# bobu36000/gym-chess

Hardware: NVIDIA B200
Metric: env_steps_per_sec (higher is better)
Workload: dtype u64

## Files before the change

__graft_entry__.py:

```python
import os
import subprocess
import sys

ROOT = os.path.dirname(os.path.abspath(__file__))
if ROOT not in sys.path:
    sys.path.insert(0, ROOT)


def build():
    from gym_chess_b200 import _lib

    _lib.build_all(force=True)
    subprocess.check_call(["make", "-C", os.path.join(ROOT, "oracle"), "-s", "-B"])
    from tests.host_emul import emul

    emul.build(force=True)
    from tests.host_emul import clone_emul

    clone_emul.build(force=True)
    import gym_chess_b200

    L = _lib.lib()
    assert L.gcb_version() >= 100


def smoke():
    import numpy as np

    from gym_chess_b200 import BatchedChessEngine, BatchedChessEnv
    from oracle import oracle as orc

    N, T, seed = 64, 40, 7
    env = BatchedChessEnv(N, opponent="none", seed=seed, device=0)
    O = [orc.OracleEnv(seed=seed, env_id=i) for i in range(N)]

    def oracle_step(i, o):
        v = o.view()
        rr, dd, _ = o.step(o.pick(orc.draw_u32(seed, i, v["episode"], v["step_in_episode"], 0)))
        if dd or o.view()["n_legal"] == 0:
            o.reset(v["episode"] + 1)
        return rr, dd

# ... 29 lines not shown
```

gym_chess_b200/csrc/chess_core.cuh:

```cuda
#pragma once
#include <stdint.h>

typedef unsigned long long u64;
typedef unsigned int u32;

#ifndef GCB_ROLL_NTH
#define GCB_ROLL_NTH 1
#endif

#if defined(__CUDACC__)
#define GCB_HD __host__ __device__ __forceinline__
#else
#define GCB_HD inline
#endif

GCB_HD u64 gcb_brev64(u64 x) {
#if defined(__CUDA_ARCH__)
    return __brevll(x);
#else
    x = ((x >> 1) & 0x5555555555555555ULL) | ((x & 0x5555555555555555ULL) << 1);
    x = ((x >> 2) & 0x3333333333333333ULL) | ((x & 0x3333333333333333ULL) << 2);
    x = ((x >> 4) & 0x0F0F0F0F0F0F0F0FULL) | ((x & 0x0F0F0F0F0F0F0F0FULL) << 4);
    return __builtin_bswap64(x);
#endif
// ... 369 lines not shown
    const u64 cand = (eRQ & (geo.line(ksq, 0) | geo.line(ksq, 1))) | (eBQ & (geo.line(ksq, 2) | geo.line(ksq, 3)));
    for (u64 p = cand; p;) {
        const int psq = gcb_take(p);
        const u64 btw = GCB_GEOM(between[ksq][psq]), blockers = btw & occ;
        if (!blockers) chk |= 1ULL << psq;
        else if (!(blockers & (blockers - 1)) && (blockers & g.own)) g.pinned |= blockers, g.pinrays |= btw | (1ULL << psq);
    }
    g.in_check = chk != 0;
    if (chk) {
        if (chk & (chk - 1)) g.cm = 0;
        else g.cm = chk | GCB_GEOM(between[ksq][gcb_lsb(chk)]);
    }
    (void)kbit;
}

GCB_HD void gen_prepare(const Board& b, int white_to_move, GenCtx& g) { gen_prepare(b, white_to_move, g, GeomGlobal()); }

GCB_HD u64 pin_mask(const GenCtx& g, int sq) {
    const u64 kbit = 1ULL << g.ksq;
    const u64 side = sq > g.ksq ? ~(kbit | (kbit - 1)) : (kbit - 1);
    return g.pinrays & line_through(g.ksq, sq) & side;
}

template <class Sink, class G>
GCB_HD void gen_targets(const Board& b, GenCtx& g, u64 subset, Sink& sink, const G& geo) {
    const u64 occ = g.occ, own = g.own, notown = ~g.own;
    const u64 mine = own & subset;
#define GCB_PUT(sq_, below_, T_)                                       \
    do {                                                               \
        const u64 t__ = (T_);                                          \
        sink.put(gcb_popc(mine & (below_)), t__);                      \
    } while (0)
    for (u64 s = bb_rooks(b) & mine; s;) {
        u64 below;
        const int sq = gcb_take(s, below);
        const u64 a = rook_att(geo, sq, occ);
        g.satt |= a;
        GCB_PUT(sq, below, a & notown & g.cm);
    }
    for (u64 s = bb_bishops(b) & mine; s;) {
        u64 below;
        const int sq = gcb_take(s, below);
        const u64 a = bishop_att(geo, sq, occ);
        g.satt |= a;
        GCB_PUT(sq, below, a & notown & g.cm);
    }
    for (u64 s = bb_queens(b) & mine; s;) {
        u64 below;
        const int sq = gcb_take(s, below);
        const u64 a = rook_att(geo, sq, occ) | bishop_att(geo, sq, occ);
        g.satt |= a;
        GCB_PUT(sq, below, a & notown & g.cm);
    }
    for (u64 s = bb_knights(b) & mine; s;) {
        u64 below;
        const int sq = gcb_take(s, below);
        const u64 a = geo.knight(sq);
        g.satt |= a;
        GCB_PUT(sq, below, a & notown & g.cm);
    }
    for (u64 s = bb_kings(b) & mine; s;) {
        u64 below;
        const int sq = gcb_take(s, below);
        const u64 a = geo.king(sq);
        g.satt |= a;
        GCB_PUT(sq, below, a & notown & ~g.eatt);
    }
    {
        const u64 pw = bb_pawns(b) & mine, allp = bb_pawns(b) & own;
        g.satt |= pawn_set_att(pw, g.white) & ~(bb_kings(b) & own);
        (void)allp;
        const u64 free_cm = ~occ & g.cm, enemy_cm = g.enemy & g.cm;
        for (u64 s = pw; s;) {
            u64 below;
            const int sq = gcb_take(s, below);
            const u64 push = geo.pawn(!g.white, sq, 0), cap = geo.pawn(!g.white, sq, 1);
            GCB_PUT(sq, below, (push & free_cm) | (cap & enemy_cm));
        }
    }
#undef GCB_PUT
    for (u64 p = g.pinned & mine & ~bb_kings(b); p;) {
        u64 below;
        const int sq = gcb_take(p, below), r = gcb_popc(mine & below);
        const u64 t = sink.get(r), t2 = t & pin_mask(g, sq);
        sink.replace(r, t, t2);
    }
}

template <class Sink>
GCB_HD void gen_targets(const Board& b, GenCtx& g, u64 subset, Sink& sink) {
    gen_targets(b, g, subset, sink, GeomGlobal());
}

GCB_HD u32 gen_castles(const Board& b, const GenCtx& g, u32 rights) {
    if (!g.has_king) return 0;
    const u64 wR = bb_rooks(b) & b.w, wK = bb_kings(b) & b.w, occ = g.occ, eatt = g.eatt;
    u32 c = 0;
    if (g.white) {
        if (!(rights & (RT_WK | RT_WQ))) return 0;
        const u64 e1 = 1ULL << 60;
        if ((wR >> 56 & 1) && !(occ & (7ULL << 57)) && (wK & e1) && !(eatt & (7ULL << 58))) c |= 1u;
        if ((wR >> 63 & 1) && !(occ & (3ULL << 61)) && (wK & e1) && !(eatt & (7ULL << 60))) c |= 2u;
    } else {
        if (!(rights & (RT_BK | RT_BQ))) return 0;
        const u64 e8 = 1ULL << 4;
        if ((wR & 1) && !(occ & (7ULL << 1)) && (wK & e8) && !(eatt & (7ULL << 2))) c |= 1u;
        if ((wR >> 7 & 1) && !(occ & (3ULL << 5)) && (wK & e8) && !(eatt & (7ULL << 4))) c |= 2u;
    }
    return c;
}
GCB_HD int castle_action(int white, int king_side) {
    return white ? (king_side ? ACT_CASTLE_KS_WHITE : ACT_CASTLE_QS_WHITE) : (king_side ? ACT_CASTLE_KS_BLACK : ACT_CASTLE_QS_BLACK);
}

// ... 426 lines not shown
```

gym_chess_b200/csrc/env_core.cuh:

```cuda
#pragma once
#include "chess_core.cuh"

#if !defined(__CUDACC__)
struct ulonglong2 {
    u64 x, y;
};
static inline ulonglong2 make_ulonglong2(u64 x, u64 y) {
    ulonglong2 r = {x, y};
    return r;
}
#endif

#if defined(__CUDACC__)
__device__ unsigned long long g_violations = 0ULL;
#endif
#if defined(GCB_CHECKED) && defined(__CUDA_ARCH__)
#define GCB_CHK(cond, code)                                                   \
    do {                                                                      \
        if (!(cond)) atomicOr(&g_violations, 1ULL << (code));                 \
    } while (0)
#else
#define GCB_CHK(cond, code) \
    do {                    \
    } while (0)
// ... 41 lines not shown
#define M_MOVECOUNT_SHIFT 22
#define M_STEP_SHIFT 38
#define M_HIST_SHIFT 54

enum { ST_STEPS = 0, ST_PLIES, ST_EPISODES, ST_MATES, ST_REPS, ST_CAPS, ST_WEDGED, ST_INVALID, ST_REWARD, ST_LEGAL,
       ST_INCHECK, ST_HISTOVF, ST_SLOTOVF, ST_HISTSCAN, ST_WINDOW, ST_USED, ST_COUNT = 16 };

struct EnvView {
    ulonglong2* bb01;
    ulonglong2* bb23;
    u64* meta;
    u64* zkey;
    u32* gen;
    ulonglong2* rep;
    u32* episode;
    ulonglong2* cnt;
    u64* tgt;
    const ulonglong2* t_bb01;
    const ulonglong2* t_bb23;
    const u64* t_meta;
    const u64* t_zkey;
    const u64* t_tgt;
    const ulonglong2* t_cnt;
    const u64* zob;
    u64* stats;
    u64* stat_rows;
    u64 seed;
    int N, slots, hist_mask, n_templates, stat_nrows;
    u32 env_offset;
    int moves_max, opponent, agent_black, auto_reset, pps;
};

struct EnvRegs {
    Board b;
    u64 zk, cnt_lo, cnt_hi;
    u32 rights, chk, castle;
    int stm_black, done, n_legal, move_count, step, hist_len, pending;
    u32 gen;
};

GCB_HD void unpack_meta(u64 m, EnvRegs& s) {
    s.stm_black = (int)(m & 1);
    s.rights = (u32)(m >> M_RIGHTS_SHIFT) & 15u;
    s.chk = (u32)(m >> 5) & 3u;
    s.done = (int)(m >> 7) & 1;
    s.castle = (u32)(m >> M_CASTLE_SHIFT) & 3u;
// ... 74 lines not shown
    }
};

struct TgtSinkFast {
    u64* base;
    unsigned N;
    int dropped;
    uint8_t* cb;
    GCB_HD TgtSinkFast(const SlotRef& sr, CountBytes* scratch) : base(sr.base), N(sr.stride), dropped(0), cb(scratch->c) {
        u64* z = reinterpret_cast<u64*>(scratch);
        z[0] = 0, z[1] = 0;
    }
    GCB_HD void put(int r, u64 t) {
        GCB_CHK((unsigned)r < 16u, CHK_SLOT_INDEX);
        base[(unsigned)r * N] = t;
        cb[r] = (uint8_t)gcb_popc(t);
    }
    GCB_HD u64 get(int r) const { return base[(unsigned)r * N]; }
    GCB_HD void replace(int r, u64, u64 tnew) {
        GCB_CHK((unsigned)r < 16u, CHK_SLOT_INDEX);
        base[(unsigned)r * N] = tnew;
        cb[r] = (uint8_t)gcb_popc(tnew);
    }
    GCB_HD u64 count_lo() const { return reinterpret_cast<const u64*>(cb)[0]; }
    GCB_HD u64 count_hi() const { return reinterpret_cast<const u64*>(cb)[1]; }
    GCB_HD int total() const {
        u64 a = count_lo(), b = count_hi();
        a = (a & 0x00FF00FF00FF00FFULL) + ((a >> 8) & 0x00FF00FF00FF00FFULL);
        b = (b & 0x00FF00FF00FF00FFULL) + ((b >> 8) & 0x00FF00FF00FF00FFULL);
        a += b;
        a += a >> 32;
        a += a >> 16;
        return (int)(a & 0xFFFF);
    }
};

struct StepStats {
    u32 f;
    int reward, legal, scan, window;
    bool wrote_slots;
    GCB_HD void clear() { f = 0, reward = 0, legal = 0, scan = 0, window = 0, wrote_slots = false; }
    GCB_HD int get(int k) const {
        switch (k) {
        case ST_STEPS: return (int)(f & 127u);
        case ST_PLIES: return (int)((f >> 7) & 255u);
        case ST_EPISODES: return (int)((f >> 22) & 1u);
        case ST_MATES: return (int)((f >> 23) & 1u);
        case ST_REPS: return (int)((f >> 24) & 1u);
        case ST_CAPS: return (int)((f >> 25) & 1u);
        case ST_WEDGED: return (int)((f >> 26) & 1u);
        case ST_INVALID: return (int)((f >> 27) & 1u);
        case ST_REWARD: return reward;
        case ST_LEGAL: return legal;
        case ST_INCHECK: return (int)((f >> 15) & 127u);
        case ST_HISTOVF: return (int)((f >> 28) & 3u);
        case ST_SLOTOVF: return (int)((f >> 30) & 3u);
        case ST_HISTSCAN: return scan;
        default: return window;
// ... 52 lines not shown
            const u64 c = (en.y & 3ULL) < 3ULL ? (en.y & 3ULL) + 1ULL : 3ULL;
            if (insert) GCB_STS(p, make_ulonglong2(key, live_tag | c));
            return (int)c;
        }
        st.scan++;
    }
    st.f += SF_HISTOVF;
    if (insert) GCB_STS(&tab[home], make_ulonglong2(key, live_tag | 1ULL));
    return 1;
}

#ifndef GCB_ONE_PICK_SITE
#define GCB_ONE_PICK_SITE 1
#endif
#ifndef GCB_SWAR_PICK
#define GCB_SWAR_PICK 1
#endif
GCB_HD u64 swar_le_u8(u64 x, u64 y) {
    const u64 H = 0x8080808080808080ULL;
    const u64 t = (y | H) - (x & ~H);
    return ((~x & y) | (~(x ^ y) & t)) & H;
}

template <bool ROLLED = true>
GCB_HD int action_at(const SlotRef& sr, const EnvRegs& s, int idx) {
    int acc = 0, hit_r = -1, hit_idx = 0;
#if GCB_SWAR_PICK
    if (s.n_legal <= 255) {
        const u64 K = 0x0101010101010101ULL;
        const u64 p_lo = s.cnt_lo * K, p_hi = (s.cnt_hi + (p_lo >> 56)) * K;
        const u64 I = (u64)(u32)idx * K;
        const int r = gcb_popc(swar_le_u8(p_lo, I)) + gcb_popc(swar_le_u8(p_hi, I));
        acc = (int)(p_hi >> 56);
        if (r < 16) {
            const u64 q = r < 8 ? (p_lo << 8) : ((p_hi << 8) | (p_lo >> 56));
            hit_r = r, hit_idx = idx - (int)((q >> (8 * (r & 7))) & 0xFF);
        }
    } else
#endif
    {
#if defined(__CUDA_ARCH__)
#pragma unroll 1
#endif
        for (int r = 0; r < 16; r++) {
            const int c = (int)(((r < 8 ? s.cnt_lo : s.cnt_hi) >> (8 * (r & 7))) & 0xFF);
            if (hit_r < 0 && idx - acc < c) hit_r = r, hit_idx = idx - acc;
            acc += c;
        }
    }
    TgtSink slots(sr, nullptr);
    u64 own = stm_pieces(s);
    if (sr.slots > 16 && hit_r < 0) {
        const int np = gcb_popc(own);
        for (int r = 16; r < np && hit_r < 0; r++) {
            const int c = gcb_popc(slots.get(r));
            if (idx - acc < c) hit_r = r, hit_idx = idx - acc;
            else acc += c;
        }
    }
    if (hit_r >= 0) {
        const u64 T = slots.get(hit_r);
        const int sq = gcb_select64(own, hit_r);
        return sq * 64 + nth_target<ROLLED>(piece_code(s.b, sq), !s.stm_black, sq, T, hit_idx);
    }
    const int king_side = (s.castle & 1u) ? (idx - acc != 0) : 1;
    return castle_action(!s.stm_black, king_side);
}

GCB_HD bool action_is_legal(const SlotRef& sr, const EnvRegs& s, int action) {
    if (action < 0) return false;
    if (action < 4096) {
        const int from = action >> 6, to = action & 63;
        const u64 own = stm_pieces(s), fbit = 1ULL << from;
        if (!(own & fbit)) return false;
        TgtSink slots(sr, nullptr);
        return (slots.get(gcb_popc(own & (fbit - 1))) >> to) & 1ULL;
    }
    if (action == castle_action(!s.stm_black, 0)) return s.castle & 1u;
    if (action == castle_action(!s.stm_black, 1)) return (s.castle >> 1) & 1u;
    return false;
}



template <bool FAST> struct SinkOf { typedef TgtSink type; };
template <> struct SinkOf<true> { typedef TgtSinkFast type; };

template <bool FAST = false, class G>
GCB_HD int ply_and_movegen(const EnvView& v, int e, EnvRegs& s, int action, bool apply, bool* rep,
                           StepStats& st, CountBytes* scratch, const SlotRef& sr, const G& geo) {
    int r = 0;
    *rep = false;
    if (apply) {
        const u64 key = hist_key(s.zk);
        u32 rights = mask_rights(s.b, s.rights);
        int status;
        bool irr;
        r = apply_action(s.b, rights, !s.stm_black, action, &status, &irr, &s.zk, v.zob);
        s.rights = rights;
        st.window += s.hist_len;
        *rep = rep_lookup_insert(v, e, s, key, !irr, st) >= 3;
        if (irr) {
            s.hist_len = 0, s.gen++;
        } else {
            if (s.hist_len < 0x1FF) s.hist_len++;
        }
    }
    s.stm_black ^= 1;
    GenCtx g;
    gen_prepare(s.b, !s.stm_black, g, geo);
    typename SinkOf<FAST>::type sink(sr, scratch);
    gen_targets(s.b, g, g.own, sink, geo);
    st.wrote_slots = true;
    const int n = sink.total();
    if (sink.dropped) st.f += SF_SLOTOVF;
    s.cnt_lo = sink.count_lo(), s.cnt_hi = sink.count_hi();
    s.castle = gen_castles(s.b, g, mask_rights(s.b, s.rights));
    s.n_legal = n + (int)(s.castle & 1u) + (int)(s.castle >> 1);
    u32 chk = g.in_check ? (1u << s.stm_black) : 0u;
    const u64 mk = bb_kings(s.b) & g.enemy;
    if (mk && ((g.satt >> ref_king_square(mk)) & 1ULL)) chk |= 1u << (s.stm_black ^ 1);
    s.chk = chk;
    return r;
}

enum { MODE_ACTION = 0, MODE_INDEX = 1, MODE_SAMPLED = 2, MODE_RESET = 3, MODE_BOTPLY = 4 };
enum { PH_AGENT = 0, PH_BOT = 1, PH_FINAL = 2, PH_RESETBOT = 3, PH_END = 4 };

struct StepIO {
    const void* in;
    int32_t* reward;
    uint8_t* done;
    uint8_t* flags;
    int32_t* act_out;
    int32_t* bot_out;
// ... 19 lines not shown

GCB_HD void env_load(const EnvView& v, int e, EnvRegs& s, u32& ep) {
    GCB_CHK((unsigned)e < (unsigned)v.N, CHK_ENV_INDEX);
    ulonglong2 a = GCB_LDS(&v.bb01[e]), c = GCB_LDS(&v.bb23[e]);
    s.b.t0 = a.x, s.b.t1 = a.y, s.b.t2 = c.x, s.b.w = c.y;
    ulonglong2 ct = GCB_LDS(&v.cnt[e]);
    s.cnt_lo = ct.x, s.cnt_hi = ct.y;
    unpack_meta(GCB_LDS(&v.meta[e]), s);
    s.zk = GCB_LDS(&v.zkey[e]);
    ep = GCB_LDS(&v.episode[e]);
    s.gen = GCB_LDS(&v.gen[e]);
}
GCB_HD void env_store(const EnvView& v, int e, const EnvRegs& s, u32 ep) {
    GCB_CHK((unsigned)e < (unsigned)v.N, CHK_ENV_INDEX);
    GCB_STS(&v.bb01[e], make_ulonglong2(s.b.t0, s.b.t1));
    GCB_STS(&v.bb23[e], make_ulonglong2(s.b.t2, s.b.w));
    GCB_STS(&v.cnt[e], make_ulonglong2(s.cnt_lo, s.cnt_hi));
    GCB_STS(&v.meta[e], pack_meta(s));
    GCB_STS(&v.zkey[e], s.zk);
    GCB_STS(&v.episode[e], ep);
    GCB_STS(&v.gen[e], s.gen);
}

template <int MODE, bool SELFPLAY = false, bool FAST = false, bool MULTI = false, class G>
GCB_HD void env_step_regs(const EnvView& v, const StepIO& io, int e, EnvRegs& s, u32& ep, StepStats& st, CountBytes* scratch,
                          const SlotRef& sr, const SlotRef& pick_sr, const G& geo, const u32 input) {
    const bool v_bot = SELFPLAY ? false : v.opponent != 0, v_ext = SELFPLAY ? false : v.opponent == 2;
    const bool v_agent_black = SELFPLAY ? false : v.agent_black != 0;
    const u32 genv = v.env_offset + (u32)e;
    int action = ACT_RESIGN, bot_action = -1, R = 0, phase;
    u32 fl = 0;
    bool d_out = false, agent_ply = false, owe_bot = false, agent_draw = false;
    const int n0 = s.n_legal;
    const bool was_done = s.done, capped = s.move_count > v.moves_max;
    const u32 step_idx = (u32)s.step;
    if (MODE == MODE_RESET) {
        phase = PH_FINAL;
    } else if (MODE == MODE_BOTPLY) {
        if (!s.pending) return;
        s.pending = 0;
        action = bot_action = (int)input;
        agent_ply = true;
        phase = (s.step == 0 && v_agent_black) ? PH_RESETBOT : PH_BOT;
    } else {
        bool valid = false;
        if (MULTI) rep_prefetch(v, e, s);
        if (MODE == MODE_ACTION) {
            action = (int)input;
            valid = action_is_legal(pick_sr, s, action);
        } else {
            if (!SELFPLAY && GCB_ONE_PICK_SITE) {
                if (n0 > 0) valid = true, agent_draw = true;
            } else {
                const u32 u = (MODE == MODE_INDEX) ? input : philox_draw(v.seed, genv, ep, step_idx, 0u);
                if (n0 > 0) {
                    action = action_at<MULTI>(pick_sr, s, (int)gcb_umulhi(u, (u32)n0));
                    valid = true;
                }
            }
        }
        const bool refused = !SELFPLAY && s.pending;
        if (refused) valid = false;
        st.f += SF_STEPS + (stm_checked(s) ? SF_INCHECK : 0u), st.legal += n0;
        if (!refused) s.step++;
        if (!valid) {
            R = -10, d_out = s.done, fl |= EF_INVALID, st.f += SF_INVALID;
            phase = PH_FINAL;
        } else if (s.done) {
            R = 0, d_out = true;
            phase = PH_FINAL;
        } else if (capped) {
            R = 0, d_out = true, fl |= EF_CAP;
            phase = PH_FINAL;
        } else {
            R = -10;
            phase = PH_AGENT;
        }
    }

    bool do_apply = true;
    int cur = action;
    u32 draw_purpose = 0u, draw_step = 0u;
#if defined(__CUDA_ARCH__)
#pragma unroll 1
#endif
    while (phase != PH_END) {
        if (!SELFPLAY && (draw_purpose || agent_draw)) {
            const u32 u = (agent_draw && MODE == MODE_INDEX) ? input : philox_draw(v.seed, genv, ep, agent_draw ? step_idx : draw_step, draw_purpose);
            cur = action_at<MULTI>(agent_draw ? pick_sr : sr, s, (int)gcb_umulhi(u, (u32)s.n_legal));
            if (agent_draw) action = cur;
            else if (draw_purpose == 1u) bot_action = cur;
            draw_purpose = 0u, agent_draw = false;
        }
        if (phase == PH_FINAL) {
            bool terminal;
            if (MODE == MODE_RESET) {
                terminal = true;
            } else {
                if (agent_ply) d_out = s.done;
                terminal = !owe_bot && (d_out || s.n_legal == 0);
                if (!owe_bot && !d_out && s.n_legal == 0) fl |= EF_WEDGED;
                if (v_ext && ((v.auto_reset && terminal) ? v_agent_black : s.pending)) fl |= EF_BOT_PENDING;
                if (n0 == 0 || was_done || owe_bot || (fl & EF_INVALID)) {
                } else if (capped) st.f += SF_CAPS;
                else if (d_out) {
                    if (fl & EF_MATE) st.f += SF_MATES;
                    else st.f += SF_REPS;
                } else if (s.n_legal == 0) st.f += SF_WEDGED;
                if (terminal) st.f += SF_EPISODES;
                st.reward += R;
                if (v.auto_reset && terminal) fl |= EF_RESET;
                GCB_CHK((unsigned)e < (unsigned)v.N, CHK_IO_INDEX);
                if (io.reward) io.reward[e] = R;
                if (io.done) io.done[e] = d_out ? 1 : 0;
                if (io.flags) io.flags[e] = (uint8_t)fl;
                if (io.packed) io.packed[e] = pack_result(R, d_out, SELFPLAY ? fl & 63u : fl);
                if (io.act_out) io.act_out[e] = action;
            }
            if ((MODE == MODE_RESET) || (v.auto_reset && terminal)) {
                const int t = (int)(genv % (u32)v.n_templates);
                ulonglong2 a = v.t_bb01[t], c = v.t_bb23[t];
                s.b.t0 = a.x, s.b.t1 = a.y, s.b.t2 = c.x, s.b.w = c.y;
                unpack_meta(v.t_meta[t], s);
                s.zk = v.t_zkey[t];
                s.gen++;
                {
                    ulonglong2 ct = v.t_cnt[t];
                    s.cnt_lo = ct.x, s.cnt_hi = ct.y;
                }
                const int np = gcb_popc(s.b.w);
                const u64* ts = v.t_tgt + (size_t)t * v.slots;
                {
                    TgtSink dst(sr, nullptr);
                    for (int r = 0; r < np && r < sr.slots; r++) dst.st(r, ts[r]);
                    st.wrote_slots = true;
                }
                ep += (u32)io.ep_inc;
                if (v_agent_black && v_ext) {
                    s.pending = 1;
                } else if (v_agent_black) {
                    if (s.n_legal > 0) {
                        draw_purpose = 2u, draw_step = 0u;
                        do_apply = true;
                    } else {
                        do_apply = false;
                    }
                    phase = PH_RESETBOT;
                    continue;
                }
            }
            phase = PH_END;
            continue;
        }
        bool rep;
        const int r = ply_and_movegen<FAST>(v, e, s, cur, do_apply, &rep, st, scratch, sr, geo);
        if (do_apply) st.f += SF_PLIES;
        const bool mate = s.n_legal == 0 && stm_checked(s);
        if (phase == PH_AGENT) {
            agent_ply = true;
            R += r;
            s.done = rep;
            if (rep) fl |= EF_REPETITION;
            if (mate) s.done = 1, R += 100, fl |= EF_MATE;
            if (!s.done && v_ext) {
                s.pending = 1, owe_bot = true;
            } else if (!s.done && v_bot) {
                if (s.n_legal > 0) {
                    draw_purpose = 1u, draw_step = step_idx;
                    phase = PH_BOT;
                    continue;
                }
            } else if (!s.done) {
                if (!s.stm_black) s.move_count++;
            }
            phase = PH_FINAL;
        } else if (phase == PH_BOT) {
            R -= r;
            s.done = rep;
// ... 62 lines not shown
}
GCB_HD bool rep_clone_entry(ulonglong2& en, u32 src_gen, u32 G) {
    const u64 c = en.y & 3ULL;
    if ((en.y >> 2) != (u64)src_gen || c == 0) return false;
    en.y = ((u64)G << 2) | c;
    return true;
}
GCB_HD void env_clone_one(const EnvView& dst, int d, const EnvView& src, int i) {
    u32 sgen;
    int hist;
    const u32 G = env_clone_words(dst, d, src, i, &sgen, &hist);
    for (int r = 0; r < dst.slots; r++) env_clone_slot(dst, d, src, i, r);
    if (hist == 0) return;
    const size_t H2 = (size_t)src.hist_mask + 1;
    const ulonglong2* from = src.rep + (size_t)i * H2;
    ulonglong2* to = dst.rep + (size_t)d * H2;
    for (size_t k = 0; k < H2; k++) {
        ulonglong2 en = GCB_LDS(&from[k]);
        if (rep_clone_entry(en, sgen, G)) GCB_STS(&to[k], en);
    }
}

GCB_HD void make_template_one(int i, const int8_t* boards, ulonglong2* bb01, ulonglong2* bb23, u64* meta, u64* zkey,
                              u64* tgt, ulonglong2* cnt, int slots) {
    Board b = board_from_mailbox(boards + (size_t)i * 64);
    EnvRegs s;
    s.b = b;
    s.zk = zobrist_full(b);
    s.rights = mask_rights(b, 15u);
    s.chk = check_flags(b);
    s.stm_black = 0, s.done = 0, s.move_count = 0, s.step = 0, s.hist_len = 0, s.pending = 0, s.gen = 0;
    GenCtx g;
    gen_prepare(b, 1, g);
    CountBytes scratch;
    SlotRef tsr = {tgt + (size_t)i * slots, 1u, slots, true};
    TgtSink sink(tsr, &scratch);
    gen_targets(b, g, g.own, sink);
    const int n = sink.total();
    s.castle = gen_castles(b, g, s.rights);
    s.n_legal = n + (int)(s.castle & 1u) + (int)(s.castle >> 1);
    cnt[i] = make_ulonglong2(sink.count_lo(), sink.count_hi());
    bb01[i] = make_ulonglong2(b.t0, b.t1);
    bb23[i] = make_ulonglong2(b.t2, b.w);
    meta[i] = pack_meta(s);
    zkey[i] = s.zk;
}

struct ListOut {
    uint16_t* out;
    int cap;
    GCB_HD void put(int pos, int action) {
        if (pos < cap) out[pos] = (uint16_t)action;
    }
};

template <class Offs, class Out>
GCB_HD int env_legal_list_one(const EnvView& v, int e, Offs& offs, Out& out, u64* stage = nullptr, unsigned stage_stride = 1) {
    EnvRegs s;
    ulonglong2 a = v.bb01[e], c = v.bb23[e];
    s.b.t0 = a.x, s.b.t1 = a.y, s.b.t2 = c.x, s.b.w = c.y;
    unpack_meta(v.meta[e], s);
    int n = 0, r0 = 0;
    u64 rem = stm_pieces(s);
    while (rem) {
        u64 chunk = rem;
        if (gcb_popc(rem) > GCB_SLOTS) {
            u64 t = rem;
            for (int i = 0; i < GCB_SLOTS; i++) t &= t - 1;
// ... 35 lines not shown
```

gym_chess_b200/csrc/gcb_kernels.cu:

```cuda
#include <cuda_runtime.h>
#include <stdint.h>
#include <stdio.h>
#include <stdlib.h>
#include <string.h>

#include <atomic>
#include <mutex>
#include <new>
#include <vector>

#include "../../include/gymchess_b200.h"
#include "env_core.cuh"

static thread_local char g_err[512] = "";
static std::atomic<uint64_t> g_launches{0};

static int fail(int code, const char* what, const char* detail) {
    snprintf(g_err, sizeof(g_err), "%s: %s", what, detail ? detail : "");
    return code;
}
#define CU(call)                                                                  \
    do {                                                                          \
        cudaError_t e_ = (call);                                                  \
        if (e_ != cudaSuccess) return fail(GCB_E_CUDA, #call, cudaGetErrorString(e_)); \
// ... 230 lines not shown
    u64 gw[(GCB_SGEOM_WORDS + GCB_BLOCK - 1) / GCB_BLOCK];
    if (TILE) {
#pragma unroll
        for (int k = 0; k < (GCB_SGEOM_WORDS + GCB_BLOCK - 1) / GCB_BLOCK; k++) {
            const int i = threadIdx.x + k * GCB_BLOCK;
            gw[k] = i < GCB_SGEOM_WORDS ? GeomShared::source_word(i) : 0ULL;
        }
    }
    u32 input = 0;
    if (active) {
        input = step_input<MODE>(io, e);
        env_load(v, e, s, ep);
    }
    if (TILE) {
#pragma unroll
        for (int k = 0; k < (GCB_SGEOM_WORDS + GCB_BLOCK - 1) / GCB_BLOCK; k++) {
            const int i = threadIdx.x + k * GCB_BLOCK;
            if (i < GCB_SGEOM_WORDS) s_geom[i] = gw[k];
        }
        __syncthreads();
    }
    const SlotRef gsr = resident_slots(v, e < io.e_end ? e : io.e_begin);
    const SlotRef tsr = {s_slots + threadIdx.x, (unsigned)GCB_BLOCK, GCB_SLOTS, true};
    if (TILE == 1 && active) {
        const int np = gcb_popc(stm_pieces(s));
        for (int r = 0; r < np && r < GCB_SLOTS; r++) s_slots[r * GCB_BLOCK + threadIdx.x] = __ldcs(gsr.base + (unsigned)r * gsr.stride);
    }
    const SlotRef sr = TILE ? tsr : gsr;
    const GeomShared sgeo = {s_geom};
    const bool small = (TILE || v.slots == GCB_SLOTS) && active && gcb_popc(s.b.w) <= GCB_SLOTS && gcb_popc(bb_occ(s.b) & ~s.b.w) <= GCB_SLOTS;
    (void)small;
    bool wrote = TILE == 1;
#pragma unroll 1
    for (int t = 0; t < nsteps; t++) {
        StepStats st;
        st.clear();
        if (active) {
            const SlotRef& pick = (TILE == 2 && !wrote) ? gsr : sr;
            if (TILE) {
#if GCB_FAST_SINK
                if (small) env_step_regs<MODE, SELFPLAY, true, TILE == 1>(v, io, e, s, ep, st, &s_counts[threadIdx.x], sr, pick, sgeo, input);
                else
#endif
                    env_step_regs<MODE, SELFPLAY, false, TILE == 1>(v, io, e, s, ep, st, &s_counts[threadIdx.x], sr, pick, sgeo, input);
            } else {
#if GCB_FAST_SINK && GCB_FAST_GENERIC
                if (small) env_step_regs<MODE, SELFPLAY, true, false>(v, io, e, s, ep, st, &s_counts[threadIdx.x], sr, pick, GeomGlobal(), input);
                else
#endif
                    env_step_regs<MODE, SELFPLAY, false, false>(v, io, e, s, ep, st, &s_counts[threadIdx.x], sr, pick, GeomGlobal(), input);
            }
            wrote = wrote || st.wrote_slots;
        }
        if (MODE != MODE_RESET) {
            const u32 f = st.f;
            const u32 hot = __reduce_add_sync(0xffffffffu, f & SF_HOT_MASK);
            const int t_reward = __reduce_add_sync(0xffffffffu, st.reward), t_legal = __reduce_add_sync(0xffffffffu, st.legal);
            const int t_scan = __reduce_add_sync(0xffffffffu, st.scan), t_window = __reduce_add_sync(0xffffffffu, st.window);
            long long mine = 0;
#define GCB_PICK(k_, v_) mine = lane == (k_) ? (long long)(v_) : mine
            GCB_PICK(ST_STEPS, hot & 127u), GCB_PICK(ST_PLIES, (hot >> 7) & 255u), GCB_PICK(ST_INCHECK, (hot >> 15) & 127u);
            GCB_PICK(ST_REWARD, t_reward), GCB_PICK(ST_LEGAL, t_legal), GCB_PICK(ST_HISTSCAN, t_scan), GCB_PICK(ST_WINDOW, t_window);
            if (__any_sync(0xffffffffu, (f >> SF_RARE_SHIFT) != 0u)) {
                const u32 r = f >> SF_RARE_SHIFT;
                const u32 w0 = (r & 1u) | ((r & 2u) << 7) | ((r & 4u) << 14) | ((r & 8u) << 21);
                const u32 w1 = ((r >> 4) & 1u) | (((r >> 5) & 1u) << 8) | (((r >> 6) & 3u) << 16) | (((r >> 8) & 3u) << 24);
                const u32 r0 = __reduce_add_sync(0xffffffffu, w0), r1 = __reduce_add_sync(0xffffffffu, w1);
                GCB_PICK(ST_EPISODES, r0 & 255u), GCB_PICK(ST_MATES, (r0 >> 8) & 255u), GCB_PICK(ST_REPS, (r0 >> 16) & 255u);
                GCB_PICK(ST_CAPS, r0 >> 24), GCB_PICK(ST_WEDGED, r1 & 255u), GCB_PICK(ST_INVALID, (r1 >> 8) & 255u);
                GCB_PICK(ST_HISTOVF, (r1 >> 16) & 255u), GCB_PICK(ST_SLOTOVF, r1 >> 24);
            }
#undef GCB_PICK
            acc += mine;
        }
        io.tick++;
        if (io.act_out) io.act_out += v.N;
        if (io.bot_out) io.bot_out += v.N;
    }
    if (active) {
        env_store(v, e, s, ep);
        if (TILE && wrote) {
            const int np = gcb_popc(stm_pieces(s));
            for (int r = 0; r < np && r < GCB_SLOTS; r++) __stcs(v.tgt + (size_t)r * v.N + e, s_slots[r * GCB_BLOCK + threadIdx.x]);
        }
    }
    if (io.bits_out) {
        u64 own = 0;
        u32 cword = 0;
        if (active) own = stm_pieces(s), cword = castle_word(s);
        write_bits_rows(io.bits_out, io.bits_stride, e - lane, io.e_end, active, e, own, cword, (TILE && wrote) ? sr : gsr, lane);
    }
    if (MODE != MODE_RESET && lane < ST_USED) {
#if !defined(GCB_SELFTEST_OOB)
        if ((e & ~31) < io.e_end)
#endif
        {
            const size_t row = (size_t)(e >> 5);
            GCB_CHK(row < (size_t)v.stat_nrows, CHK_STAT_ROW);
            atomicAdd(reinterpret_cast<unsigned long long*>(v.stat_rows + row * ST_COUNT + lane), (unsigned long long)acc);
        }
    }
}

template <int MODE, int TILE = 0, bool SELFPLAY = false>
__global__ void __launch_bounds__(GCB_BLOCK, (MODE == MODE_SAMPLED && TILE == 1) ? GCB_SAMPLED_MIN_BLOCKS : GCB_STEP_MIN_BLOCKS)
    k_env_step(EnvView v, StepIO io) {
    __shared__ CountBytes s_counts[GCB_BLOCK];
    __shared__ u64 s_slots[TILE ? GCB_SLOTS * GCB_BLOCK : 1];
    __shared__ u64 s_geom[TILE ? GCB_SGEOM_WORDS : 1];
    run_unit<MODE, TILE, SELFPLAY>(v, io, io.e_begin + blockIdx.x * GCB_BLOCK + threadIdx.x, MODE == MODE_SAMPLED ? io.nsteps : 1,
                                   s_slots, s_geom, s_counts);
}

__global__ void k_stats_reduce(const u64* __restrict__ rows, int nrows, u64* __restrict__ out) {
    __shared__ u64 s[32][ST_COUNT + 1];
    const int k = threadIdx.x & 15, part = threadIdx.x >> 4;
    u64 acc = 0;
    for (int r = part; r < nrows; r += 32) acc += rows[(size_t)r * ST_COUNT + k];
    s[part][k] = acc;
    __syncthreads();
    if (threadIdx.x < ST_COUNT) {
        u64 t = 0;
        for (int p = 0; p < 32; p++) t += s[p][threadIdx.x];
        out[threadIdx.x] = t;
    }
}

__global__ void k_make_templates(int n, const int8_t* __restrict__ boards, ulonglong2* bb01, ulonglong2* bb23, u64* meta,
                                 u64* zkey, u64* tgt, ulonglong2* cnt, int slots) {
    int i = blockIdx.x * blockDim.x + threadIdx.x;
    if (i >= n) return;
    make_template_one(i, boards, bb01, bb23, meta, zkey, tgt, cnt, slots);
}

__global__ void __launch_bounds__(GCB_BLOCK) k_env_import(EnvView v, const int8_t* __restrict__ boards,
                                                          const int8_t* __restrict__ players, const uint8_t* __restrict__ rights4,
                                                          const int32_t* __restrict__ move_count, const uint8_t* __restrict__ mask,
                                                          u64 tick) {
    __shared__ CountBytes s_counts[GCB_BLOCK];
    const int e = blockIdx.x * blockDim.x + threadIdx.x;
    if (e >= v.N) return;
    if (mask && !mask[e]) return;
    alignas(16) int8_t m[64];
    const int4* src = reinterpret_cast<const int4*>(boards + (size_t)e * 64);
#pragma unroll
    for (int k = 0; k < 4; k++) *reinterpret_cast<int4*>(m + 16 * k) = __ldg(src + k);
    const uchar4 q = reinterpret_cast<const uchar4*>(rights4)[e];
    const u32 rights = (q.x ? RT_WK : 0) | (q.y ? RT_WQ : 0) | (q.z ? RT_BK : 0) | (q.w ? RT_BQ : 0);
    StepStats st;
    st.clear();
    env_import_one(v, e, m, players[e], rights, move_count ? move_count[e] : 0, st, &s_counts[threadIdx.x]);
}

#define GCB_CLONE_BATCH 8
__global__ void __launch_bounds__(GCB_BLOCK) k_env_clone(EnvView dst, EnvView src, const int32_t* __restrict__ index,
// ... 296 lines not shown
    CU(cudaMemcpyAsync(d_b, boards, (size_t)n * 64, cudaMemcpyHostToDevice, 0));
    CU(cudaMemcpyAsync(d_r, rights4, (size_t)n * 4, cudaMemcpyHostToDevice, 0));
    if (int rc = gcb_pack(n, d_b, nullptr, d_r, pos, 0)) return rc;
    if (int rc = gcb_update_state(n, pos, d_or, d_oc, 0)) return rc;
    uint8_t* tmp = new (std::nothrow) uint8_t[2 * (size_t)n];
    if (!tmp) return fail(GCB_E_NOMEM, "new", "host scratch");
    cudaError_t e1 = cudaMemcpy(tmp, d_or, n, cudaMemcpyDeviceToHost);
    cudaError_t e2 = cudaMemcpy(tmp + n, d_oc, n, cudaMemcpyDeviceToHost);
    for (int i = 0; i < n; i++) {
        uint8_t r = tmp[i], c = tmp[n + i];
        out_rights4[4 * i] = r & 1, out_rights4[4 * i + 1] = (r >> 1) & 1, out_rights4[4 * i + 2] = (r >> 2) & 1,
                        out_rights4[4 * i + 3] = (r >> 3) & 1;
        out_checks[2 * i] = c & 1, out_checks[2 * i + 1] = (c >> 1) & 1;
    }
    delete[] tmp;
    if (e1 != cudaSuccess || e2 != cudaSuccess) return fail(GCB_E_CUDA, "cudaMemcpy", "update_state results");
    return GCB_OK;
}

struct gcb_env {
    gcb_env_config cfg;
    EnvView v;
    ulonglong2 *t_bb01 = nullptr, *t_bb23 = nullptr;
    u64 *t_meta = nullptr, *t_zkey = nullptr, *t_tgt = nullptr, *zob = nullptr;
    ulonglong2* t_cnt = nullptr;
    u64 tick = 0;
    int32_t *d_in = nullptr, *d_reward = nullptr;
    uint8_t *d_done = nullptr, *d_flags = nullptr;
    cudaStream_t streams[8] = {nullptr, nullptr, nullptr, nullptr, nullptr, nullptr, nullptr, nullptr};
    cudaEvent_t events[9] = {nullptr, nullptr, nullptr, nullptr, nullptr, nullptr, nullptr, nullptr, nullptr};
    struct Alloc {
        const char* name;
        char* base;
        char* user;
        size_t bytes;
    };
    std::vector<Alloc> allocs;
    size_t guard = 0;
    u64* bits_out = nullptr;
    int bits_stride = 0;
};
#define GCB_GUARD_BYTE 0xA5

static cudaError_t env_alloc(gcb_env* env, const char* name, void** out, size_t bytes) {
    const size_t G = env->guard;
    char* base = nullptr;
    cudaError_t e = cudaMalloc((void**)&base, bytes + 2 * G + (G ? 256 : 0));
// ... 108 lines not shown
    EnvView& v = env->v;
    memset(&v, 0, sizeof(v));
    int8_t* d_tb = nullptr;
    cudaError_t e = cudaSuccess;
#define ALLOC(ptr, bytes) \
    if (e == cudaSuccess) e = env_alloc(env, #ptr, (void**)&(ptr), (bytes))
    ALLOC(v.bb01, (size_t)N * 16);
    ALLOC(v.bb23, (size_t)N * 16);
    ALLOC(v.meta, (size_t)N * 8);
    ALLOC(v.zkey, (size_t)N * 8);
    ALLOC(v.gen, (size_t)N * 4);
    ALLOC(v.cnt, (size_t)N * 16);
    ALLOC(env->t_cnt, (size_t)T * 16);
    ALLOC(v.episode, (size_t)N * 4);
    ALLOC(v.tgt, (size_t)N * S * 8);
    ALLOC(v.rep, (size_t)N * 2 * H * 16);
    ALLOC(v.stats, ST_COUNT * 8);
    ALLOC(v.stat_rows, (size_t)((N + 31) / 32) * ST_COUNT * 8);
    ALLOC(env->t_bb01, (size_t)T * 16);
    ALLOC(env->t_bb23, (size_t)T * 16);
    ALLOC(env->t_meta, (size_t)T * 8);
    ALLOC(env->t_zkey, (size_t)T * 8);
    ALLOC(env->t_tgt, (size_t)T * S * 8);
    ALLOC(env->zob, (size_t)GCB_ZOB_ENTRIES * 8);
    ALLOC(env->d_in, (size_t)N * 4);
    ALLOC(env->d_reward, (size_t)N * 4);
    ALLOC(env->d_done, (size_t)N);
    ALLOC(env->d_flags, (size_t)N);
#undef ALLOC
    if (e == cudaSuccess) e = cudaMalloc((void**)&d_tb, (size_t)T * 64);
    if (e != cudaSuccess) {
        cudaFree(d_tb);
        gcb_env_destroy(env);
        return fail(GCB_E_NOMEM, "cudaMalloc", cudaGetErrorString(e));
    }
    v.t_bb01 = env->t_bb01, v.t_bb23 = env->t_bb23, v.t_meta = env->t_meta, v.t_zkey = env->t_zkey, v.t_tgt = env->t_tgt;
    v.zob = env->zob, v.t_cnt = env->t_cnt;
    v.seed = cfg.seed, v.N = N, v.slots = S, v.hist_mask = 2 * H - 1, v.n_templates = T, v.env_offset = cfg.env_id_offset;
    v.stat_nrows = (N + 31) / 32;
    v.moves_max = cfg.moves_max, v.opponent = cfg.opponent, v.agent_black = cfg.agent_black, v.auto_reset = cfg.auto_reset;
    v.pps = 1 + (cfg.opponent == 1 ? 1 : 0);
    int rc = GCB_OK;
    do {
        if (cudaMemcpy(d_tb, cfg.n_templates > 0 ? cfg.template_boards : kDefaultBoard, (size_t)T * 64, cudaMemcpyHostToDevice) !=
                cudaSuccess ||
            cudaMemset(v.stats, 0, ST_COUNT * 8) != cudaSuccess ||
            cudaMemset(v.stat_rows, 0, (size_t)((N + 31) / 32) * ST_COUNT * 8) != cudaSuccess || cudaMemset(v.episode, 0, (size_t)N * 4) != cudaSuccess ||
            cudaMemset(v.meta, 0, (size_t)N * 8) != cudaSuccess || cudaMemset(v.bb01, 0, (size_t)N * 16) != cudaSuccess ||
            cudaMemset(v.bb23, 0, (size_t)N * 16) != cudaSuccess || cudaMemset(v.zkey, 0, (size_t)N * 8) != cudaSuccess ||
            cudaMemset(v.gen, 0, (size_t)N * 4) != cudaSuccess || cudaMemset(v.rep, 0, (size_t)N * 2 * H * 16) != cudaSuccess || cudaMemset(v.cnt, 0, (size_t)N * 16) != cudaSuccess || cudaMemset(v.tgt, 0, (size_t)N * S * 8) != cudaSuccess ||
            cudaMemset(env->t_tgt, 0, (size_t)T * S * 8) != cudaSuccess) {
            rc = fail(GCB_E_CUDA, "cudaMemcpy/cudaMemset", "env init");
            break;
        }
        k_init_zobrist<<<(GCB_ZOB_ENTRIES + 127) / 128, 128>>>(env->zob);
        k_make_templates<<<(T + 63) / 64, 64>>>(T, d_tb, env->t_bb01, env->t_bb23, env->t_meta, env->t_zkey, env->t_tgt, env->t_cnt, S);
        g_launches.fetch_add(2);
        StepIO io;
        memset(&io, 0, sizeof(io));
        io.tick = env->tick, io.e_begin = 0, io.e_end = N, io.nsteps = 1;
        k_env_step<MODE_RESET, 0, false><<<grid_for(N), GCB_BLOCK>>>(v, io);
        env->tick++;
        g_launches.fetch_add(1);
        cudaError_t e2 = cudaDeviceSynchronize();
        if (e2 != cudaSuccess) rc = fail(GCB_E_CUDA, "env init kernels", cudaGetErrorString(e2));
    } while (0);
    cudaFree(d_tb);
    if (rc) {
        gcb_env_destroy(env);
        return rc;
    }
    *out = env;
    return GCB_OK;
}

#define ENV_CHECK(env)                                               \
    if (!(env)) return fail(GCB_E_ARG, __func__, "null env");        \
    DeviceScope dev_scope_;                                          \
    CU(dev_scope_.enter((env)->cfg.device))
// ... 469 lines not shown
```

Before: 8.787 billion.

## Represent pawn moves as four direction bitboards in shared-memory tile path

In the tiled fast-sink sampled path, pawn move generation no longer loops over pawns to write per-square target slots. It computes four whole-board bitboards (push, double push, two captures) with shifts, derives per-square counts with bit-sliced adders, and stores the bitboards in extra shared-memory tile words. Action selection decodes pawn moves from these bitboards, and the boards are converted back to slot form at kernel exit and derived from slots at entry. This adds shared memory per block (which may lower occupancy) plus conversion work at entry and exit, in exchange for cheaper per-ply pawn generation.

```diff
diff --git a/__graft_entry__.py b/__graft_entry__.py
--- a/__graft_entry__.py
+++ b/__graft_entry__.py
@@ -18,6 +18,9 @@
     from tests.host_emul import clone_emul
 
     clone_emul.build(force=True)
+    from tests.host_emul import tile_emul
+
+    tile_emul.build(force=True)
     import gym_chess_b200
 
     L = _lib.lib()
diff --git a/gym_chess_b200/csrc/chess_core.cuh b/gym_chess_b200/csrc/chess_core.cuh
--- a/gym_chess_b200/csrc/chess_core.cuh
+++ b/gym_chess_b200/csrc/chess_core.cuh
@@ -415,7 +415,7 @@
     return g.pinrays & line_through(g.ksq, sq) & side;
 }
 
-template <class Sink, class G>
+template <bool PAWN_SLOTS = true, class Sink, class G>
 GCB_HD void gen_targets(const Board& b, GenCtx& g, u64 subset, Sink& sink, const G& geo) {
     const u64 occ = g.occ, own = g.own, notown = ~g.own;
     const u64 mine = own & subset;
@@ -459,7 +459,7 @@
         g.satt |= a;
         GCB_PUT(sq, below, a & notown & ~g.eatt);
     }
-    {
+    if (PAWN_SLOTS) {
         const u64 pw = bb_pawns(b) & mine, allp = bb_pawns(b) & own;
         g.satt |= pawn_set_att(pw, g.white) & ~(bb_kings(b) & own);
         (void)allp;
@@ -472,7 +472,7 @@
         }
     }
 #undef GCB_PUT
-    for (u64 p = g.pinned & mine & ~bb_kings(b); p;) {
+    for (u64 p = g.pinned & mine & ~bb_kings(b) & (PAWN_SLOTS ? ~0ULL : ~bb_pawns(b)); p;) {
         u64 below;
         const int sq = gcb_take(p, below), r = gcb_popc(mine & below);
         const u64 t = sink.get(r), t2 = t & pin_mask(g, sq);
@@ -483,6 +483,40 @@
 template <class Sink>
 GCB_HD void gen_targets(const Board& b, GenCtx& g, u64 subset, Sink& sink) {
     gen_targets(b, g, subset, sink, GeomGlobal());
+}
+
+GCB_HD int pawn_to(int white, int sq, int k) {
+    return white ? sq - (int)((0x09071008u >> (8 * k)) & 0xFFu) : sq + (int)((0x07091008u >> (8 * k)) & 0xFFu);
+}
+#define GCB_ROW1 0x000000000000FF00ULL
+#define GCB_ROW6 0x00FF000000000000ULL
+GCB_HD void gen_pawn_boards(const Board& b, GenCtx& g, u64 d[4]) {
+    const u64 pw = bb_pawns(b) & g.own;
+    g.satt |= pawn_set_att(pw, g.white) & ~(bb_kings(b) & g.own);
+    const u64 free_cm = ~g.occ & g.cm, enemy_cm = g.enemy & g.cm;
+    if (g.white) {
+        d[0] = pw & (free_cm << 8), d[1] = pw & GCB_ROW6 & (free_cm << 16);
+        d[2] = pw & ~GCB_FILE_H & (enemy_cm << 7), d[3] = pw & ~GCB_FILE_A & (enemy_cm << 9);
+    } else {
+        d[0] = pw & (free_cm >> 8), d[1] = pw & GCB_ROW1 & (free_cm >> 16);
+        d[2] = pw & ~GCB_FILE_H & (enemy_cm >> 9), d[3] = pw & ~GCB_FILE_A & (enemy_cm >> 7);
+    }
+    for (u64 p = g.pinned & pw; p;) {
+        const int sq = gcb_take(p);
+        const u64 keep = pin_mask(g, sq), bit = 1ULL << sq;
+        for (int k = 0; k < 4; k++)
+            if (!(keep & sq_bit_safe(pawn_to(g.white, sq, k)))) d[k] &= ~bit;
+    }
+}
+template <class Sink>
+GCB_HD void put_pawn_counts(const GenCtx& g, const u64 d[4], Sink& sink) {
+    const u64 x = d[0] ^ d[1], y = d[2] ^ d[3];
+    const u64 c0 = x ^ y, c1 = (d[0] & d[1]) ^ (d[2] & d[3]) ^ (x & y), c2 = d[0] & d[1] & d[2] & d[3];
+    for (u64 m = d[0] | d[1] | d[2] | d[3]; m;) {
+        u64 below;
+        const int sq = gcb_take(m, below);
+        sink.count(gcb_popc(g.own & below), (int)((c0 >> sq) & 1ULL) + 2 * (int)((c1 >> sq) & 1ULL) + 4 * (int)((c2 >> sq) & 1ULL));
+    }
 }
 
 GCB_HD u32 gen_castles(const Board& b, const GenCtx& g, u32 rights) {
diff --git a/gym_chess_b200/csrc/env_core.cuh b/gym_chess_b200/csrc/env_core.cuh
--- a/gym_chess_b200/csrc/env_core.cuh
+++ b/gym_chess_b200/csrc/env_core.cuh
@@ -87,6 +87,7 @@
     const u64* t_zkey;
     const u64* t_tgt;
     const ulonglong2* t_cnt;
+    const u64* t_pawnb;
     const u64* zob;
     u64* stats;
     u64* stat_rows;
@@ -207,6 +208,10 @@
         base[(unsigned)r * N] = tnew;
         cb[r] = (uint8_t)gcb_popc(tnew);
     }
+    GCB_HD void count(int r, int c) {
+        GCB_CHK((unsigned)r < 16u, CHK_SLOT_INDEX);
+        cb[r] = (uint8_t)c;
+    }
     GCB_HD u64 count_lo() const { return reinterpret_cast<const u64*>(cb)[0]; }
     GCB_HD u64 count_hi() const { return reinterpret_cast<const u64*>(cb)[1]; }
     GCB_HD int total() const {
@@ -219,6 +224,40 @@
         return (int)(a & 0xFFFF);
     }
 };
+
+#define GCB_TILE_WORDS (GCB_SLOTS + 4)
+GCB_HD u64 pawn_board(const SlotRef& tile, int k) {
+    GCB_CHK((unsigned)k < 4u, CHK_SLOT_INDEX);
+    return tile.base[(unsigned)(GCB_SLOTS + k) * tile.stride];
+}
+GCB_HD void set_pawn_board(const SlotRef& tile, int k, u64 d) {
+    GCB_CHK((unsigned)k < 4u, CHK_SLOT_INDEX);
+    tile.base[(unsigned)(GCB_SLOTS + k) * tile.stride] = d;
+}
+GCB_HD void pawn_boards_from_slots(const Board& b, int white, const SlotRef& slots, u64 d[4]) {
+    const u64 own = white ? b.w : (bb_occ(b) & ~b.w), pawns = bb_pawns(b) & own;
+    const TgtSink from(slots, nullptr);
+    d[0] = d[1] = d[2] = d[3] = 0;
+    for (u64 p = pawns; p; p &= p - 1) {
+        const int sq = gcb_lsb(p);
+        const u64 T = from.get(gcb_popc(own & ((1ULL << sq) - 1)));
+        for (int k = 0; k < 4; k++)
+            if (T & sq_bit_safe(pawn_to(white, sq, k))) d[k] |= 1ULL << sq;
+    }
+}
+GCB_HD void pawn_slots_from_boards(const Board& b, int white, const SlotRef& tile) {
+    const u64 own = white ? b.w : (bb_occ(b) & ~b.w), pawns = bb_pawns(b) & own;
+    u64 d[4];
+    for (int k = 0; k < 4; k++) d[k] = pawn_board(tile, k);
+    TgtSink to(tile, nullptr);
+    for (u64 p = pawns; p; p &= p - 1) {
+        const int sq = gcb_lsb(p);
+        u64 T = 0;
+        for (int k = 0; k < 4; k++)
+            if ((d[k] >> sq) & 1ULL) T |= 1ULL << pawn_to(white, sq, k);
+        to.st(gcb_popc(own & ((1ULL << sq) - 1)), T);
+    }
+}
 
 struct StepStats {
     u32 f;
@@ -317,7 +356,7 @@
     return ((~x & y) | (~(x ^ y) & t)) & H;
 }
 
-template <bool ROLLED = true>
+template <bool ROLLED = true, bool PAWNB = false>
 GCB_HD int action_at(const SlotRef& sr, const EnvRegs& s, int idx) {
     int acc = 0, hit_r = -1, hit_idx = 0;
 #if GCB_SWAR_PICK
@@ -355,8 +394,13 @@
     }
     if (hit_r >= 0) {
         const u64 T = slots.get(hit_r);
-        const int sq = gcb_select64(own, hit_r);
-        return sq * 64 + nth_target<ROLLED>(piece_code(s.b, sq), !s.stm_black, sq, T, hit_idx);
+        const int sq = gcb_select64(own, hit_r), code = piece_code(s.b, sq);
+        if (PAWNB && code == PC_PAWN) {
+            const int c0 = (int)(pawn_board(sr, 0) >> sq) & 1, c1 = c0 + ((int)(pawn_board(sr, 1) >> sq) & 1),
+                      c2 = c1 + ((int)(pawn_board(sr, 2) >> sq) & 1);
+            return sq * 64 + pawn_to(!s.stm_black, sq, (int)(hit_idx >= c0) + (int)(hit_idx >= c1) + (int)(hit_idx >= c2));
+        }
+        return sq * 64 + nth_target<ROLLED>(code, !s.stm_black, sq, T, hit_idx);
     }
     const int king_side = (s.castle & 1u) ? (idx - acc != 0) : 1;
     return castle_action(!s.stm_black, king_side);
@@ -381,7 +425,7 @@
 template <bool FAST> struct SinkOf { typedef TgtSink type; };
 template <> struct SinkOf<true> { typedef TgtSinkFast type; };
 
-template <bool FAST = false, class G>
+template <bool FAST = false, bool PAWNB = false, class G>
 GCB_HD int ply_and_movegen(const EnvView& v, int e, EnvRegs& s, int action, bool apply, bool* rep,
                            StepStats& st, CountBytes* scratch, const SlotRef& sr, const G& geo) {
     int r = 0;
@@ -405,7 +449,15 @@
     GenCtx g;
     gen_prepare(s.b, !s.stm_black, g, geo);
     typename SinkOf<FAST>::type sink(sr, scratch);
-    gen_targets(s.b, g, g.own, sink, geo);
+    if constexpr (PAWNB) {
+        gen_targets<false>(s.b, g, g.own, sink, geo);
+        u64 d[4];
+        gen_pawn_boards(s.b, g, d);
+        for (int k = 0; k < 4; k++) set_pawn_board(sr, k, d[k]);
+        put_pawn_counts(g, d, sink);
+    } else {
+        gen_targets(s.b, g, g.own, sink, geo);
+    }
     st.wrote_slots = true;
     const int n = sink.total();
     if (sink.dropped) st.f += SF_SLOTOVF;
@@ -471,7 +523,7 @@
     GCB_STS(&v.gen[e], s.gen);
 }
 
-template <int MODE, bool SELFPLAY = false, bool FAST = false, bool MULTI = false, class G>
+template <int MODE, bool SELFPLAY = false, bool FAST = false, bool MULTI = false, bool PAWNB = false, class G>
 GCB_HD void env_step_regs(const EnvView& v, const StepIO& io, int e, EnvRegs& s, u32& ep, StepStats& st, CountBytes* scratch,
                           const SlotRef& sr, const SlotRef& pick_sr, const G& geo, const u32 input) {
     const bool v_bot = SELFPLAY ? false : v.opponent != 0, v_ext = SELFPLAY ? false : v.opponent == 2;
@@ -503,7 +555,7 @@
             } else {
                 const u32 u = (MODE == MODE_INDEX) ? input : philox_draw(v.seed, genv, ep, step_idx, 0u);
                 if (n0 > 0) {
-                    action = action_at<MULTI>(pick_sr, s, (int)gcb_umulhi(u, (u32)n0));
+                    action = action_at<MULTI, PAWNB>(pick_sr, s, (int)gcb_umulhi(u, (u32)n0));
                     valid = true;
                 }
             }
@@ -536,7 +588,7 @@
     while (phase != PH_END) {
         if (!SELFPLAY && (draw_purpose || agent_draw)) {
             const u32 u = (agent_draw && MODE == MODE_INDEX) ? input : philox_draw(v.seed, genv, ep, agent_draw ? step_idx : draw_step, draw_purpose);
-            cur = action_at<MULTI>(agent_draw ? pick_sr : sr, s, (int)gcb_umulhi(u, (u32)s.n_legal));
+            cur = action_at<MULTI, PAWNB>(agent_draw ? pick_sr : sr, s, (int)gcb_umulhi(u, (u32)s.n_legal));
             if (agent_draw) action = cur;
             else if (draw_purpose == 1u) bot_action = cur;
             draw_purpose = 0u, agent_draw = false;
@@ -582,6 +634,10 @@
                 {
                     TgtSink dst(sr, nullptr);
                     for (int r = 0; r < np && r < sr.slots; r++) dst.st(r, ts[r]);
+                    if (PAWNB) {
+                        GCB_CHK((unsigned)t < (unsigned)v.n_templates, CHK_SLOT_INDEX);
+                        for (int k = 0; k < 4; k++) set_pawn_board(sr, k, v.t_pawnb[(size_t)t * 4 + k]);
+                    }
                     st.wrote_slots = true;
                 }
                 ep += (u32)io.ep_inc;
@@ -602,7 +658,7 @@
             continue;
         }
         bool rep;
-        const int r = ply_and_movegen<FAST>(v, e, s, cur, do_apply, &rep, st, scratch, sr, geo);
+        const int r = ply_and_movegen<FAST, PAWNB>(v, e, s, cur, do_apply, &rep, st, scratch, sr, geo);
         if (do_apply) st.f += SF_PLIES;
         const bool mate = s.n_legal == 0 && stm_checked(s);
         if (phase == PH_AGENT) {
@@ -711,7 +767,7 @@
 }
 
 GCB_HD void make_template_one(int i, const int8_t* boards, ulonglong2* bb01, ulonglong2* bb23, u64* meta, u64* zkey,
-                              u64* tgt, ulonglong2* cnt, int slots) {
+                              u64* tgt, ulonglong2* cnt, int slots, u64* pawnb = nullptr) {
     Board b = board_from_mailbox(boards + (size_t)i * 64);
     EnvRegs s;
     s.b = b;
@@ -733,6 +789,7 @@
     bb23[i] = make_ulonglong2(b.t2, b.w);
     meta[i] = pack_meta(s);
     zkey[i] = s.zk;
+    if (pawnb) pawn_boards_from_slots(b, 1, tsr, pawnb + (size_t)i * 4);
 }
 
 struct ListOut {
diff --git a/gym_chess_b200/csrc/gcb_kernels.cu b/gym_chess_b200/csrc/gcb_kernels.cu
--- a/gym_chess_b200/csrc/gcb_kernels.cu
+++ b/gym_chess_b200/csrc/gcb_kernels.cu
@@ -276,14 +276,19 @@
     }
     const SlotRef gsr = resident_slots(v, e < io.e_end ? e : io.e_begin);
     const SlotRef tsr = {s_slots + threadIdx.x, (unsigned)GCB_BLOCK, GCB_SLOTS, true};
+    const bool small = (TILE || v.slots == GCB_SLOTS) && active && gcb_popc(s.b.w) <= GCB_SLOTS && gcb_popc(bb_occ(s.b) & ~s.b.w) <= GCB_SLOTS;
+    (void)small;
     if (TILE == 1 && active) {
         const int np = gcb_popc(stm_pieces(s));
         for (int r = 0; r < np && r < GCB_SLOTS; r++) s_slots[r * GCB_BLOCK + threadIdx.x] = __ldcs(gsr.base + (unsigned)r * gsr.stride);
+        if (GCB_FAST_SINK && small) {
+            u64 d[4];
+            pawn_boards_from_slots(s.b, !s.stm_black, tsr, d);
+            for (int k = 0; k < 4; k++) set_pawn_board(tsr, k, d[k]);
+        }
     }
     const SlotRef sr = TILE ? tsr : gsr;
     const GeomShared sgeo = {s_geom};
-    const bool small = (TILE || v.slots == GCB_SLOTS) && active && gcb_popc(s.b.w) <= GCB_SLOTS && gcb_popc(bb_occ(s.b) & ~s.b.w) <= GCB_SLOTS;
-    (void)small;
     bool wrote = TILE == 1;
 #pragma unroll 1
     for (int t = 0; t < nsteps; t++) {
@@ -293,7 +298,7 @@
             const SlotRef& pick = (TILE == 2 && !wrote) ? gsr : sr;
             if (TILE) {
 #if GCB_FAST_SINK
-                if (small) env_step_regs<MODE, SELFPLAY, true, TILE == 1>(v, io, e, s, ep, st, &s_counts[threadIdx.x], sr, pick, sgeo, input);
+                if (small) env_step_regs<MODE, SELFPLAY, true, TILE == 1, TILE == 1>(v, io, e, s, ep, st, &s_counts[threadIdx.x], sr, pick, sgeo, input);
                 else
 #endif
                     env_step_regs<MODE, SELFPLAY, false, TILE == 1>(v, io, e, s, ep, st, &s_counts[threadIdx.x], sr, pick, sgeo, input);
@@ -333,6 +338,7 @@
     }
     if (active) {
         env_store(v, e, s, ep);
+        if (TILE == 1 && GCB_FAST_SINK && small) pawn_slots_from_boards(s.b, !s.stm_black, tsr);
         if (TILE && wrote) {
             const int np = gcb_popc(stm_pieces(s));
             for (int r = 0; r < np && r < GCB_SLOTS; r++) __stcs(v.tgt + (size_t)r * v.N + e, s_slots[r * GCB_BLOCK + threadIdx.x]);
@@ -360,7 +366,7 @@
 __global__ void __launch_bounds__(GCB_BLOCK, (MODE == MODE_SAMPLED && TILE == 1) ? GCB_SAMPLED_MIN_BLOCKS : GCB_STEP_MIN_BLOCKS)
     k_env_step(EnvView v, StepIO io) {
     __shared__ CountBytes s_counts[GCB_BLOCK];
-    __shared__ u64 s_slots[TILE ? GCB_SLOTS * GCB_BLOCK : 1];
+    __shared__ u64 s_slots[TILE == 1 ? GCB_TILE_WORDS * GCB_BLOCK : TILE ? GCB_SLOTS * GCB_BLOCK : 1];
     __shared__ u64 s_geom[TILE ? GCB_SGEOM_WORDS : 1];
     run_unit<MODE, TILE, SELFPLAY>(v, io, io.e_begin + blockIdx.x * GCB_BLOCK + threadIdx.x, MODE == MODE_SAMPLED ? io.nsteps : 1,
                                    s_slots, s_geom, s_counts);
@@ -381,10 +387,10 @@
 }
 
 __global__ void k_make_templates(int n, const int8_t* __restrict__ boards, ulonglong2* bb01, ulonglong2* bb23, u64* meta,
-                                 u64* zkey, u64* tgt, ulonglong2* cnt, int slots) {
+                                 u64* zkey, u64* tgt, ulonglong2* cnt, int slots, u64* pawnb) {
     int i = blockIdx.x * blockDim.x + threadIdx.x;
     if (i >= n) return;
-    make_template_one(i, boards, bb01, bb23, meta, zkey, tgt, cnt, slots);
+    make_template_one(i, boards, bb01, bb23, meta, zkey, tgt, cnt, slots, pawnb);
 }
 
 __global__ void __launch_bounds__(GCB_BLOCK) k_env_import(EnvView v, const int8_t* __restrict__ boards,
@@ -727,7 +733,7 @@
     gcb_env_config cfg;
     EnvView v;
     ulonglong2 *t_bb01 = nullptr, *t_bb23 = nullptr;
-    u64 *t_meta = nullptr, *t_zkey = nullptr, *t_tgt = nullptr, *zob = nullptr;
+    u64 *t_meta = nullptr, *t_zkey = nullptr, *t_tgt = nullptr, *zob = nullptr, *t_pawnb = nullptr;
     ulonglong2* t_cnt = nullptr;
     u64 tick = 0;
     int32_t *d_in = nullptr, *d_reward = nullptr;
@@ -882,6 +888,7 @@
     ALLOC(env->t_meta, (size_t)T * 8);
     ALLOC(env->t_zkey, (size_t)T * 8);
     ALLOC(env->t_tgt, (size_t)T * S * 8);
+    ALLOC(env->t_pawnb, (size_t)T * 4 * 8);
     ALLOC(env->zob, (size_t)GCB_ZOB_ENTRIES * 8);
     ALLOC(env->d_in, (size_t)N * 4);
     ALLOC(env->d_reward, (size_t)N * 4);
@@ -895,7 +902,7 @@
         return fail(GCB_E_NOMEM, "cudaMalloc", cudaGetErrorString(e));
     }
     v.t_bb01 = env->t_bb01, v.t_bb23 = env->t_bb23, v.t_meta = env->t_meta, v.t_zkey = env->t_zkey, v.t_tgt = env->t_tgt;
-    v.zob = env->zob, v.t_cnt = env->t_cnt;
+    v.zob = env->zob, v.t_cnt = env->t_cnt, v.t_pawnb = env->t_pawnb;
     v.seed = cfg.seed, v.N = N, v.slots = S, v.hist_mask = 2 * H - 1, v.n_templates = T, v.env_offset = cfg.env_id_offset;
     v.stat_nrows = (N + 31) / 32;
     v.moves_max = cfg.moves_max, v.opponent = cfg.opponent, v.agent_black = cfg.agent_black, v.auto_reset = cfg.auto_reset;
@@ -914,7 +921,7 @@
             break;
         }
         k_init_zobrist<<<(GCB_ZOB_ENTRIES + 127) / 128, 128>>>(env->zob);
-        k_make_templates<<<(T + 63) / 64, 64>>>(T, d_tb, env->t_bb01, env->t_bb23, env->t_meta, env->t_zkey, env->t_tgt, env->t_cnt, S);
+        k_make_templates<<<(T + 63) / 64, 64>>>(T, d_tb, env->t_bb01, env->t_bb23, env->t_meta, env->t_zkey, env->t_tgt, env->t_cnt, S, env->t_pawnb);
         g_launches.fetch_add(2);
         StepIO io;
         memset(&io, 0, sizeof(io));
```

Result: slower. 7.495 billion, median of 6 (-14.7%).
